# blyssprivacy/sdk

Measured on AMD Instinct MI355X. Metric: PIR queries/sec (full answer path) on 2^20 items x 256 B, higher is better.
Workload: dtype u64; 1 GPU; spiral-rs process_query, c2 = {"db_item_size": 256, "instances": 1, "n": 2, "nu_1": 9, "nu_2": 11, "p": 256, "q2_bits": 20, "t_conv": 4, "t_exp_left": 8, "t_exp_right": 56, "t_gsw": 8}, encoded DB 64.0 GiB (56.0 GiB resident per GPU), unsharded, one query per step

## Files before the change

### sdk_amd/csrc/capi.cpp

```cpp
#include <chrono>
#include <cstdlib>
#include <cstring>
#include <deque>
#include <new>

#include "../../include/spiral_hip.h"
#include "pipeline.hpp"

using namespace spiral;

static thread_local std::string g_last_error;
static thread_local int g_last_rc = SP_OK;

template <typename F>
static int guarded(F&& f) {
  tunables_new_call();
  auto fail = [](int rc, const char* what) {
    g_last_error = what;
    g_last_rc = rc;
    return rc;
  };
  try {
    f();
    g_last_rc = SP_OK;
// ... 226 lines not shown
  }
  auto idx = std::make_shared<SparseIndex>();
  idx->col_ptr.ensure(ptr.size());
  idx->col_rows.ensure(std::max<size_t>(rows.size(), 1));
  idx->col_slots.ensure(std::max<size_t>(slots.size(), 1));
  upload_words(idx->col_ptr.p, ptr.data(), ptr.size() * sizeof(int));
  if (!rows.empty()) {
    upload_words(idx->col_rows.p, rows.data(), rows.size() * sizeof(int));
    upload_words(idx->col_slots.p, slots.data(), slots.size() * sizeof(int));
  }
  if (slots_cap == 0) polys.ensure(1);
  if (rows_dirty || !sparse_index || !sparse_index->plan)
    idx->plan = build_pruned_plan_rows(p, row_set);
  else
    idx->plan = sparse_index->plan;
  sparse_index = idx;
  index_dirty = false;
  rows_dirty = false;
  return sparse_index;
}

extern "C" {

const char* sp_last_error(void) { return g_last_error.c_str(); }

uint64_t sp_paths_taken(int reset) { return paths_taken(reset != 0); }
int sp_debug_set(const char* name, long value) {
  if (!name) return SP_E_ARG;
  set_tunable(name, value);
  return SP_OK;
}
static thread_local int g_shard_split_hint = 1;
extern "C" void sp_shard_split_hint_(int on) { g_shard_split_hint = on; }
extern "C" int sp_scatter_group_choice_(const sp_db_t* db, int G) {
  if (!db || !db->packed || db->col_G != 1 || db->sparse || db->num_shards != G) return 1;
  SweepBatchDesc d{};
  d.batch = SWEEP_BATCH_MAX;
  d.num_per = db->np_local;
  d.nj = db->nj;
  tunables_new_call();
  return sweep_batch_scatter_ok(d, G) && G <= (int)tunable("batch_scatter_max_g", BATCH_SCATTER_MAX_G_DEFAULT) ? SWEEP_BATCH_MAX : 1;
}
void sp_set_last_error_(const char* msg) { g_last_error = msg ? msg : ""; }
void sp_note_path_(uint64_t bits) { note_path(bits); }

const char* sp_path_name(int bit) {
  static const char* names[] = {"sweep_packed_persist", "sweep_packed", "sweep_wide", "sweep_narrow", "sweep_batch",
                                "from_sweep4", "from_sweep1", "fold_fused", "fold_tail_delta", "fold_tail_literal",
                                "pipelined_fold_overlap", "expand_pruned", "pack_v1", "direct_upload", "scatter_out",
                                "from_sweep4_xcd_order", "fold_tail_persistent", "expand_round_one_launch", "sweep_sparse",
                                "rccl_in_library", "fold_wave", "cu_split_overlap", "expand_split", "pipe_class_split",
                                "sweep_batch_mfma", "custom_transport", "from_sweep_wave",
                                "fold_tail_batched", "sweep_ring", "sweep_batch_mfma_two_tiles", "fold_wave8", "sweep_batch_planar",
                                "expand_group", "expand_wave", "sweep_batch_scatter"};
  return bit >= 0 && bit < (int)(sizeof(names) / sizeof(names[0])) ? names[bit] : nullptr;
}

int sp_device_count(void) {
  int n = 0;
  if (hipGetDeviceCount(&n) != hipSuccess) {
    (void)hipGetLastError();
    return 0;
  }
  return n;
}
int sp_set_device(int device) {
  return guarded([&] { HIP_CHECK(hipSetDevice(device)); });
}

sp_params_t* sp_params_from_json(const char* json) {
  sp_params_t* out = nullptr;
  int rc = guarded([&] {
    need(json != nullptr, "json is null");
    auto h = std::make_unique<sp_params>();
    h->p = Params::from_json(json);
    out = h.release();
  });
  return rc == SP_OK ? out : nullptr;
}
void sp_params_free(sp_params_t* p) { delete p; }

uint64_t sp_params_get(const sp_params_t* h, const char* name) {
  if (!h || !name) return UINT64_MAX;
  const Params& p = h->p;
  std::string s(name);
  if (s == "poly_len") return p.poly_len;
  if (s == "poly_len_log2") return p.poly_len_log2;
  if (s == "crt_count") return p.crt_count;
  if (s == "modulus") return p.modulus;
  if (s == "modulus_log2") return p.modulus_log2;
  if (s == "moduli0") return p.moduli[0];
  if (s == "moduli1") return p.moduli[1];
  if (s == "n") return p.n;
  if (s == "pt_modulus") return p.pt_modulus;
  if (s == "q2_bits") return p.q2_bits;
  if (s == "t_conv") return p.t_conv;
  if (s == "t_exp_left") return p.t_exp_left;
  if (s == "t_exp_right") return p.t_exp_right;
  if (s == "t_gsw") return p.t_gsw;
  if (s == "expand_queries") return p.expand_queries;
  if (s == "db_dim_1") return p.db_dim_1;
  if (s == "db_dim_2") return p.db_dim_2;
  if (s == "instances") return p.instances;
  if (s == "db_item_size") return p.db_item_size;
  if (s == "version") return p.version;
  if (s == "g") return p.g();
  if (s == "stop_round") return p.stop_round();
// ... 1353 lines not shown
    join_right(*W);
    download_raw(*W, W->qv.p, POLY_LEN * p.dim0() * 2, v_reg_reoriented);
    const size_t nu2 = p.db_dim_2, two_t = 2 * p.t_gsw;
    if (nu2 > 0) {
      need(v_folding != nullptr, "v_folding is null");
      DevBuf<u32> dense(nu2 * 2 * two_t * 2 * POLY_LEN);
      for (size_t d = 0; d < nu2; d++)
        for (size_t r = 0; r < 2; r++)
          HIP_CHECK(hipMemcpyAsync(dense.p + ((d * 2 + r) * two_t) * 2 * POLY_LEN,
                                   W->fold_mats.p + ((d * 2 + r) * 2 * two_t + two_t) * 2 * POLY_LEN,
                                   two_t * 2 * POLY_LEN * sizeof(u32), hipMemcpyDeviceToDevice, W->stream));
      DevBuf<u64> tmp;
      download_ntt(*W, dense.p, nu2 * 2 * two_t * 2 * POLY_LEN, v_folding, tmp);
    }
  });
}

int sp_fold_ciphertexts(const sp_params_t* h, uint64_t* cts, size_t num_per, const uint64_t* v_folding,
                        const uint64_t* v_folding_neg) {
  return guarded([&] {
    need(h && cts && v_folding && v_folding_neg, "null argument");
    const Params& p = h->p;
    need(num_per >= 1 && (num_per & (num_per - 1)) == 0, "num_per must be a power of two");
    size_t further = 0;
    while (((size_t)1 << further) < num_per) further++;
    if (further == 0) return;
    const size_t two_t = 2 * p.t_gsw;
    Scoped W(h);
    ensure_stage_fold(*W, num_per, further);
    DevBuf<u64> tmp;
    DevBuf<u32> dF, dFn;
    upload_ntt(*W, v_folding, further * 2 * two_t * 2 * POLY_LEN, dF, tmp);
    DevBuf<u64> tmp2;
    upload_ntt(*W, v_folding_neg, further * 2 * two_t * 2 * POLY_LEN, dFn, tmp2);
    for (size_t d = 0; d < further; d++)
      for (size_t r = 0; r < 2; r++) {
        u32* row = W->fold_mats.p + ((d * 2 + r) * 2 * two_t) * 2 * POLY_LEN;
        HIP_CHECK(hipMemcpyAsync(row, dFn.p + ((d * 2 + r) * two_t) * 2 * POLY_LEN, two_t * 2 * POLY_LEN * sizeof(u32), hipMemcpyDeviceToDevice, W->stream));
        HIP_CHECK(hipMemcpyAsync(row + two_t * 2 * POLY_LEN, dF.p + ((d * 2 + r) * two_t) * 2 * POLY_LEN, two_t * 2 * POLY_LEN * sizeof(u32), hipMemcpyDeviceToDevice, W->stream));
      }
    HIP_CHECK(hipMemcpyAsync(W->foldX.p, cts, num_per * 2 * POLY_LEN * 8, hipMemcpyHostToDevice, W->stream));
    W->mats_w_ready = false;
    u64* res = run_fold(*W, FoldOpts{1L << 60, false, false}, W->foldX.p, W->foldY.p, 1, (int)num_per, -1);
    download_raw(*W, res, 2 * POLY_LEN, cts);
  });
}

int sp_fold_ciphertexts_fused(const sp_params_t* h, uint64_t* cts, size_t num_per, const uint64_t* v_folding,
                              long fused_min_pairs) {
  return guarded([&] {
    need(h && cts && v_folding, "null argument");
    const Params& p = h->p;
    need(num_per >= 1 && (num_per & (num_per - 1)) == 0, "num_per must be a power of two");
    size_t further = 0;
    while (((size_t)1 << further) < num_per) further++;
    if (further == 0) return;
    const size_t two_t = 2 * p.t_gsw;
    Scoped W(h);
    ensure_stage_fold(*W, num_per, further);
    DevBuf<u64> tmp;
    DevBuf<u32> dF;
    upload_ntt(*W, v_folding, further * 2 * two_t * 2 * POLY_LEN, dF, tmp);
    for (size_t d = 0; d < further; d++)
      for (size_t r = 0; r < 2; r++) {
        u32* row = W->fold_mats.p + ((d * 2 + r) * 2 * two_t) * 2 * POLY_LEN;
        HIP_CHECK(hipMemcpyAsync(row + two_t * 2 * POLY_LEN, dF.p + ((d * 2 + r) * two_t) * 2 * POLY_LEN, two_t * 2 * POLY_LEN * sizeof(u32), hipMemcpyDeviceToDevice, W->stream));
      }
    launch_folding_neg(W->D->T, W->fold_mats.p, W->D->gadget_gsw.p, (int)further, (int)two_t, W->stream);
    run_mats_to_wave(*W, further);
    HIP_CHECK(hipMemcpyAsync(W->foldX.p, cts, num_per * 2 * POLY_LEN * 8, hipMemcpyHostToDevice, W->stream));
    bool below_q = true;
    for (size_t i = 0; i < num_per * 2 * POLY_LEN && below_q; i++) below_q = cts[i] < p.modulus;
    const FoldOpts o{fused_min_pairs > 0 ? fused_min_pairs : W->fused_min_pairs, true, below_q};
    u64* res = run_fold(*W, o, W->foldX.p, W->foldY.p, 1, (int)num_per, -1);
    download_raw(*W, res, 2 * POLY_LEN, cts);
  });
}

int sp_pack(const sp_params_t* h, const sp_pp_t* pp, const uint64_t* v_ct, uint64_t* out) {
  return guarded([&] {
    need(h && pp && v_ct && out, "null argument");
    const Params& p = h->p;
    need(p.instances == 1, "sp_pack packs one instance (n*n cts); call per instance");
    check_device(pp->device);
    Scoped W(h);
    W->ensure_finish();
    HIP_CHECK(hipMemcpyAsync(W->final_cts.p, v_ct, p.n * p.n * 2 * POLY_LEN * 8, hipMemcpyHostToDevice, W->stream));
    run_pack(*W, *pp);
    DevBuf<u64> tmp;
    download_ntt(*W, W->pack_res.p, (p.n + 1) * p.n * 2 * POLY_LEN, out, tmp);
  });
}

int sp_encode(const sp_params_t* h, const uint64_t* v_packed, uint8_t* out, size_t out_cap, size_t* out_len) {
  return guarded([&] {
    need(h && v_packed && out && out_len, "null argument");
    need(out_cap >= h->p.response_bytes(), "output buffer smaller than response_bytes");
    *out_len = encode_response(h->p, v_packed, out);
  });
}

}
```

### sdk_amd/csrc/fold.hip

```cpp
#include <type_traits>

#include "device_common.hpp"
#include "wave_ntt.hpp"
#include "bodies.hpp"

namespace spiral {

__device__ __forceinline__ bool fold_zero_shortcut(const u64* ct0, const u64* ct1, u64* out, int tau) {
  int nz0 = 0, nz1 = 0;
#pragma unroll
  for (int k = 0; k < 16; k++) {
    nz0 |= ct0[tau + 256 * k] != 0;
    nz1 |= ct1[tau + 256 * k] != 0;
  }
  const int any0 = __syncthreads_or(nz0), any1 = __syncthreads_or(nz1);
  if (any0 && any1) return false;
  const u64* src = any0 ? ct0 : ct1;
#pragma unroll
  for (int k = 0; k < 16; k++) out[tau + 256 * k] = src[tau + 256 * k];
  return true;
}

__global__ __launch_bounds__(256, 2) void k_fold_fused(DevTables T, FoldDesc d) {
  __shared__ u32 lds0[LDS_WORDS];
  __shared__ u32 lds1[LDS_WORDS];
  const int tau = threadIdx.x;
  const int i = (int)blockIdx.x, plane = blockIdx.y;
  const int two_t = 2 * d.t, four_t = 4 * d.t;
  const int t_live = d.t_live > 0 && d.t_live < d.t ? d.t_live : d.t;
  const u64* ct0 = d.X + ((size_t)plane * d.cur + i) * 2 * N;
  const u64* ct1 = ct0 + (size_t)d.half * 2 * N;
  const u64 mask = (1ULL << d.bits) - 1ULL;
  u32* la = lds0;
  u32* lb = lds1;
  u64* out = d.Y + ((size_t)plane * d.half + i) * 2 * N;
  if (d.zero_shortcuts && fold_zero_shortcut(ct0, ct1, out, tau)) return;
#pragma unroll 1
  for (int c = 0; c < 2; c++) {
    const ModConst m = T.c.mod[c];
    const u32* fw = T.tw + (size_t)c * 4 * N;
    u64 acc0[8], acc1[8];
#pragma unroll
    for (int k = 0; k < 8; k++) acc0[k] = acc1[k] = 0;
#pragma unroll 1
    for (int j = 0; j < 2; j++) {
      u64 x0[8], x1[8];
#pragma unroll
      for (int k = 0; k < 8; k++) {
        x0[k] = ct0[(size_t)j * N + tau + 256 * k];
        x1[k] = ct1[(size_t)j * N + tau + 256 * k];
      }
#pragma unroll 1
// ... 371 lines not shown
#pragma unroll
        for (int k = 0; k < 32; k++) rr[k] = wv == 0 ? r0[k] : r1[k];
      } else {
#pragma unroll
        for (int g = 0; g < 8; g++) {
          const u32x4w_t t4 = *reinterpret_cast<const u32x4w_t*>(park + irow * N + g * 256 + 4 * lt);
          rr[4 * g] = t4.x; rr[4 * g + 1] = t4.y; rr[4 * g + 2] = t4.z; rr[4 * g + 3] = t4.w;
        }
      }
      const int khalf = wv >> 1;
      const u64* crow = ct0 + (size_t)irow * N + (size_t)khalf * 1024;
      u64 cpre[16];
#pragma unroll
      for (int kk = 0; kk < 16; kk++) cpre[kk] = crow[64 * kk + lt];
      wntt_inv(rr, lt, mybuf, inv_tables(T.tw, imod), mi.q, mi.two_q);
      u32* exch = smem_fw + 4 * WBUF_WORDS;
      u32* mine_out = exch + (irow * 2 + imod) * (N / 2);
      if (wv < 2) {
#pragma unroll
        for (int kk = 0; kk < 16; kk++) mine_out[64 * kk + lt] = rr[16 + kk];
      } else {
#pragma unroll
        for (int kk = 0; kk < 16; kk++) mine_out[64 * kk + lt] = rr[kk];
      }
      __syncthreads();
      {
        const u32* theirs = exch + (irow * 2 + (1 - imod)) * (N / 2);
        u64* orow = out + (size_t)irow * N + (size_t)khalf * 1024;
        const u32 q0 = T.c.mod[0].q, q1 = T.c.mod[1].q;
        auto compose = [&](auto mod1_wave) {
          constexpr bool M1 = decltype(mod1_wave)::value;
#pragma unroll
          for (int kk = 0; kk < 16; kk++) {
            const u32 other = theirs[64 * kk + lt];
            const u32 own = rr[M1 ? kk : 16 + kk];
            const u32 x = M1 ? other : own, y = M1 ? own : other;
            const u32 xm = x >= q1 ? x - q1 : x;
            const u32 dd = y >= xm ? y - xm : y + q1 - xm;
            const u32 qt = __umulhi(dd, T.c.q0_inv_q1_sh);
            u32 e = dd * T.c.q0_inv_q1 - qt * q1;
            e = e >= q1 ? e - q1 : e;
            const u64 val = (u64)x + (u64)q0 * (u64)e + cpre[kk];
            const u64 res = val >= T.c.Q ? val - T.c.Q : val;
            orow[64 * kk + lt] = res;
          }
        };
        if (wv < 2) compose(std::true_type{});
        else compose(std::false_type{});
      }
    }
  }
}

__global__ __launch_bounds__(256, 2) void k_expand_wave(DevTables T, ExpandWaveDesc d, GroupOff g) {
  extern __shared__ __attribute__((aligned(16))) u32 smem_fw[];
  u32* wbuf = smem_fw;
  u32* ltw = smem_fw + 4 * WBUF_WORDS;
  u64* raw0 = reinterpret_cast<u64*>(ltw + 2 * N);
  const int tau = threadIdx.x, lane = tau & 63;
  const int wv = __builtin_amdgcn_readfirstlane(tau >> 6);
  const int b = (int)blockIdx.x, c = (int)blockIdx.y, qi = (int)blockIdx.z;
  const ModConst m = T.c.mod[c];
  const u32* fw = T.tw + (size_t)c * 4 * N;
  const u64* src = group_rebase(d.raw, g.raw[qi]) + (size_t)d.pos[b] * 2 * N;
  const u32* A_w = group_rebase(d.A_w, g.pp[qi]);
  u32* vout = group_rebase(d.v, g.v[qi]);
  u32* mybuf = wbuf + wv * WBUF_WORDS;
  wtw_stage(ltw, wave_fwd_image(T.tw, c), tau);
#pragma unroll
  for (int k = 0; k < 8; k++) raw0[tau + 256 * k] = src[tau + 256 * k];
  __syncthreads();
  const u64 mask = (1ULL << d.bits) - 1ULL;
  u64 acc0[32], acc1[32];
#pragma unroll
  for (int k = 0; k < 32; k++) acc0[k] = acc1[k] = 0;
#pragma unroll 1
  for (int dg = wv; dg <= d.t; dg += 4) {
    int ln = lane;
    const u32* fwi = fw;
    asm volatile("" : "+v"(ln));
    asm volatile("" : "+s"(fwi));
    WaveScalarTw stw;
    wntt_scalar_tw(stw, fwi);
    u32 v[32];
    if (dg < d.t) {
      const int sh = dg * d.bits;
#pragma unroll
      for (int k = 0; k < 32; k++) v[k] = sh < 64 ? (u32)((raw0[64 * k + ln] >> (sh & 63)) & mask) : 0u;
    } else {
#pragma unroll
      for (int k = 0; k < 32; k++) v[k] = reduce64(src[(size_t)N + 64 * k + ln], m);
    }
    SP_SB();
    const u32* a0 = dg < d.t ? A_w + ((size_t)dg * 2 + c) * N : d.const_w;
    const u32* a1 = dg < d.t ? A_w + ((size_t)(d.t + dg) * 2 + c) * N : d.const_w + N;
    FoldMac hk{acc0, acc1, reinterpret_cast<const u32x4w_t*>(a0) + ln, reinterpret_cast<const u32x4w_t*>(a1) + ln};
    wntt_fwd<false>(v, ln, mybuf, fwi, stw, ltw, m.q, m.two_q, hk);
  }
  int lt = lane;
  asm volatile("" : "+v"(lt));
  u32 r0[32], r1[32];
#pragma unroll
  for (int k = 0; k < 32; k++) {
    r0[k] = reduce64(acc0[k], m);
    r1[k] = reduce64(acc1[k], m);
  }
// ... 97 lines not shown
```

### sdk_amd/csrc/kernels.hpp

```cpp
#pragma once
#include <hip/hip_runtime.h>

#include <vector>

#include "params.hpp"

namespace spiral {

constexpr int N = (int)POLY_LEN;

struct DevTables {
  const u32* tw;
  DevConsts c;
};
__host__ __device__ inline const u32* inv_tables(const u32* tw, int c) { return tw + (size_t)8 * N + (size_t)c * 2 * N; }
__host__ __device__ inline const u32* wave_fwd_image(const u32* tw, int c) { return tw + (size_t)12 * N + (size_t)c * 2 * N; }
__host__ __device__ inline int wtw_phys(int idx) {
  if (idx >= 1024) {
    const int L = (idx - 1024) >> 4, r = (idx - 1024) & 15;
    return 1024 + 16 * L + 4 * (((r >> 2) + (L >> 2)) & 3) + (r & 3);
  }
  if (idx >= 512) {
    const int L = (idx - 512) >> 3, r = (idx - 512) & 7;
    return 512 + 8 * L + 4 * (((r >> 2) + (L >> 3)) & 1) + (r & 3);
  }
  return idx;
}

enum PathBit : u64 {
  PATH_SWEEP_PERSIST = 1ull << 0,
  PATH_SWEEP_PACKED = 1ull << 1,
  PATH_SWEEP_WIDE = 1ull << 2,
  PATH_SWEEP_NARROW = 1ull << 3,
  PATH_SWEEP_BATCH = 1ull << 4,
  PATH_FROM_SWEEP4 = 1ull << 5,
  PATH_FROM_SWEEP1 = 1ull << 6,
  PATH_FOLD_FUSED = 1ull << 7,
  PATH_FOLD_TAIL = 1ull << 8,
  PATH_FOLD_TAIL_LITERAL = 1ull << 9,
  PATH_PIPELINED = 1ull << 10,
  PATH_EXPAND_PRUNED = 1ull << 11,
  PATH_PACK_V1 = 1ull << 12,
  PATH_DIRECT_UPLOAD = 1ull << 13,
  PATH_SCATTER_OUT = 1ull << 14,
  PATH_SWEEP_XCD_FROM = 1ull << 15,
  PATH_FOLD_TAIL_PERSIST = 1ull << 16,
  PATH_EXPAND_FUSED = 1ull << 17,
  PATH_SWEEP_SPARSE = 1ull << 18,
  PATH_RCCL = 1ull << 19,
  PATH_FOLD_WAVE = 1ull << 20,
  PATH_CU_SPLIT = 1ull << 21,
  PATH_EXPAND_SPLIT = 1ull << 22,
  PATH_PIPE_CLASS_SPLIT = 1ull << 23,
  PATH_SWEEP_MFMA = 1ull << 24,
  PATH_CUSTOM_TRANSPORT = 1ull << 25,
  PATH_FROM_SWEEP_WAVE = 1ull << 26,
  PATH_FOLD_TAIL_BATCHED = 1ull << 27,
  PATH_SWEEP_RING = 1ull << 28,
  PATH_SWEEP_MFMA2 = 1ull << 29,
  PATH_FOLD_WAVE8 = 1ull << 30,
  PATH_SWEEP_PLANAR = 1ull << 31,
  PATH_EXPAND_GROUP = 1ull << 32,
  PATH_EXPAND_WAVE = 1ull << 33,
  PATH_SWEEP_BATCH_SCATTER = 1ull << 34
};
long tunable(const char* name, long dflt);
void launched(u64 path_bits, const char* kernel);
void note_path(u64 path_bits);
void launch_checksum(const u32* p, size_t n_words, unsigned long long* out, hipStream_t s);
void launch_cache_sync(u32* sink, hipStream_t s);
void launch_copy_words(u32* dst, const u32* src, size_t n_words, hipStream_t s);
void debug_stage(int stage);

struct FwdDesc {
  const u64* src;
  const int* src_idx;
  u32* dst;
  int n_out;
  int rdim, cols, t, bits;
  int src_batch_stride;
  int src_row0, src_cols;
  long delta_off;
  int delta_inner, delta_outer_stride;
};
void launch_ntt_fwd(const DevTables& T, const FwdDesc& d, hipStream_t s);
void launch_ntt_fwd3(const DevTables& T, const FwdDesc& d0, const FwdDesc& d1, const FwdDesc& d2, hipStream_t s);

float bench_ntt_core(const DevTables& T, int M, int blocks, int reps, u32* scratch, hipStream_t s);

struct InvDesc {
  const u32* src;
  const int* idx;
  int polys_per_idx;
  long idx_stride, poly_stride, crt_stride, z_stride;
  u64* dst;
  int n_polys;
  int premod;
  int sweep_np;
  int automorph_t;
  const u32* scal;
  u32* scal_dst;
  int scal_thresh;
  const int* scal_only_idx;
  int n_scalar_only;
  const u64* addend;
  int add_inner2, add_outer_stride;
};
void launch_ntt_inv(const DevTables& T, const InvDesc& d, hipStream_t s);
void launch_from_sweep4(const DevTables& T, const u32* src, int np, int n_planes, int premod, u64* dst, hipStream_t s);

struct MacDesc {
  const u32* A;
  const u32* B;
  u32* out;
  const u32* addend;
  const int* out_idx;
  int R, K;
// ... 13 lines not shown
struct ExpandSideDesc {
  const u64* raw;
  const int* pos;
  const int* out_idx;
  const u32* A;
  u32* v;
  int cnt, t, bits;
};
void launch_expand_round(const DevTables& T, const ExpandSideDesc& left, const ExpandSideDesc& right, hipStream_t s);
constexpr long EXPAND_ROUND_MIN_DEFAULT = 2048;

constexpr int GROUP_MAX = 16;
struct GroupOff {
  long long v[GROUP_MAX], raw[GROUP_MAX], dig[GROUP_MAX], ct1[GROUP_MAX], pp[GROUP_MAX];
};
void launch_ntt_inv_group(const DevTables& T, const InvDesc& d, const GroupOff& g, int B, hipStream_t s);
void launch_ntt_fwd3_group(const DevTables& T, const FwdDesc& d0, const FwdDesc& d1, const FwdDesc& d2, const GroupOff& g, int B,
                           hipStream_t s);
void launch_mac2_group(const DevTables& T, const MacDesc& d0, const MacDesc& d1, const GroupOff& g, int B, hipStream_t s);
void launch_expand_round_group(const DevTables& T, const ExpandSideDesc& left, const ExpandSideDesc& right, const GroupOff& g, int B,
                               hipStream_t s);
void launch_reorient_group(u64* out, const u32* v, int first, int step, int dim0, const GroupOff& g, int B, hipStream_t s);
void launch_copy_polys_group(u32* dst, const int* dst_idx, int dst_row_stride, const u32* src, const int* src_idx, int src_row_stride,
                             int R, int batch, const GroupOff& g, int B, hipStream_t s);
void launch_folding_neg_group(const DevTables& T, u32* mats, const u32* gadget_ntt, int nu2, int two_t, const GroupOff& g, int B,
                              hipStream_t s);
void launch_mats_to_wave_group(u32* dst, const u32* src, size_t n_words, int half_polys, const GroupOff& g, int B, hipStream_t s);
struct ExpandWaveDesc {
  const u64* raw;
  const int* pos;
  const int* out_idx;
  const u32* A_w;
  const u32* const_w;
  u32* v;
  int cnt, t, bits;
};
void launch_expand_wave(const DevTables& T, const ExpandWaveDesc& d, const GroupOff& g, int B, hipStream_t s);
constexpr long EXPAND_WAVE_MIN_DIGITS_DEFAULT = 16;
constexpr long EXPAND_GROUP_ROUND_MIN_DEFAULT = 4096;

struct FoldDesc {
  const u64* X;
  u64* Y;
  const u32* mats;
  int cur, half, planes;
  int t, bits;
  int t_live;
  int zero_shortcuts;
  const u32* mats_w;
};
void launch_mats_to_wave(u32* dst, const u32* src, size_t n_words, hipStream_t s, int half_polys = 0);
constexpr long FOLD_VARIANT_DEFAULT = 5;
void launch_fold_fused(const DevTables& T, const FoldDesc& d, hipStream_t s);

void launch_add_poly_into(const DevTables& T, u32* dst, const int* idx, const u32* src, int batch, hipStream_t s);
void launch_scalar_mul(const DevTables& T, u32* base, long dst_off, long src_off, const u32* scalar, int n_polys,
                       hipStream_t s);
void launch_add_polys_idx(const DevTables& T, u32* dst, const int* di, const u32* a, const int* ai, const u32* b,
                          const int* bi, int count, hipStream_t s);
void launch_interleave_query(u64* qv, const u32* row0_ntt, const u64* wire, int dim0, hipStream_t s);
void launch_copy_polys(u32* dst, const int* dst_idx, int dst_row_stride, const u32* src, const int* src_idx,
                       int src_row_stride, int R, int batch, hipStream_t s);
void launch_folding_neg(const DevTables& T, u32* mats, const u32* gadget_ntt, int nu2, int two_t, hipStream_t s);
void launch_add(const DevTables& T, u32* out, const u32* a, const u32* b, int n_polys, hipStream_t s);
void launch_invert_raw(const DevTables& T, u64* out, const u64* a, long n_words, hipStream_t s);
void launch_automorph(const DevTables& T, u64* out, const u64* a, int n_polys, int t, hipStream_t s);
void launch_gadget_raw(u64* out, const u64* inp, int rows_in, int cols, int rows_out, int rdim, int bits,
                       hipStream_t s);
void launch_u64_to_u32(u32* out, const u64* in, long n, hipStream_t s);
void launch_u32_to_u64(u64* out, const u32* in, long n, hipStream_t s);

void launch_cu_probe(u32* out, int blocks, hipStream_t s);

struct EncodeDesc {
  const u64* packed;
  unsigned long long* out;
  int instances, n;
  u64 Q, q1, q2;
  int q1_bits, q2_bits;
};
void launch_encode(const EncodeDesc& d, hipStream_t s);

void launch_reorient(u64* out, const u32* v, int first, int step, int dim0, hipStream_t s);

struct CopyPolysDesc {
  u32* dst;
  const int* dst_idx;
  int dst_row_stride;
  const u32* src;
  const int* src_idx;
  int src_row_stride, R, batch;
};
struct FoldingNegDesc {
  u32* mats;
  const u32* gadget_ntt;
  int two_t, nu2;
};
struct ReorientDesc {
  u64* out;
  const u32* v;
  int first, step, dim0;
};
struct MatsToWaveDesc {
  u32* dst;
  const u32* src;
  size_t n_words;
// ... 103 lines not shown
```

### sdk_amd/csrc/pipeline.hpp

```cpp
#pragma once
#include <vector>

#include "server.hpp"

namespace spiral {

struct Workspace {
  const Params* P;
  DeviceState* D;
  int device = -1;
  hipStream_t stream = nullptr;
  hipStream_t stream2 = nullptr;
  std::vector<hipEvent_t> ev_plane;
  hipEvent_t ev_fold = nullptr;
  hipEvent_t ev_round0 = nullptr, ev_right = nullptr;
  bool right_pending = false;
  bool long_sweep_follows = false;
  hipEvent_t ev_sw[2] = {nullptr, nullptr};
  bool have_sweep_span = false;
  bool pipelined = false;
  hipEvent_t ev[5] = {nullptr, nullptr, nullptr, nullptr, nullptr};
  DevBuf<u64> q_raw;
  DevBuf<u32> v;
  DevBuf<u64> exp_raw;
// ... 9 lines not shown
  DevBuf<u32> gsw_dig;
  DevBuf<u32> sweep_out;
  DevBuf<u64> fold_tail;
  DevBuf<u32> batch_rq;
  DevBuf<u64> foldX, foldY, final_cts, pack_raw;
  DevBuf<u32> fold_dig, fold_ntt, pack_dig, pack_ct2, pack_res, pack_v1_P, pack_v1_P2;
  DevBuf<u64> pack_v1_raw, du_raw, du_wire;
  DevBuf<u32> du_ntt;
  u64* h_query = nullptr;
  u64* h_group_query = nullptr;
  DevBuf<u64> group_q_raw;
  u64* h_packed = nullptr;
  size_t h_packed_words = 0;
  DevBuf<u64> enc_out;
  uint8_t* h_response = nullptr;
  bool host_pinned = true;
  int out_G = 1;
  bool zero_shortcuts = false;
  long fused_min_pairs = 256;

  Workspace(const Params& P, DeviceState& D);
  ~Workspace();
  Workspace(const Workspace&) = delete;
  Workspace& operator=(const Workspace&) = delete;
  void ensure_expand();
  void ensure_sweep();
  void ensure_finish();
  size_t plane_group() const;
};

void run_coefficient_expansion(Workspace& W, const sp_pp& pp, size_t g_rounds, const DeviceState::PrunedPlan* plan = nullptr,
                               int tree = 0, size_t r_begin = 0);
void join_right(Workspace& W);
void run_regev_to_gsw(Workspace& W, const sp_pp& pp, const u32* v_src, const int* src_ct, const int* src_poly);
void run_folding_neg(Workspace& W);
void run_mats_to_wave(Workspace& W, size_t levels, bool c_only = false);
void run_fold_operands(Workspace& W);
void run_begin_direct(Workspace& W, const uint8_t* query);
void run_begin_group(Workspace* const* Ws, const sp_pp* const* pps, const uint8_t* const* queries, const size_t* query_lens, int B);
void run_begin(Workspace& W, const sp_pp& pp, const uint8_t* query, size_t query_len, int j0 = 0, int nj = 0,
               const DeviceState::PrunedPlan* plan = nullptr);
void run_sweep_sparse(Workspace& W, const sp_db& db, const int* col_ptr, const int* col_rows, const int* col_slots);
std::unique_ptr<DeviceState::PrunedPlan> build_pruned_plan_rows(const Params& P, const std::vector<char>& rows);
void run_sweep(Workspace& W, const sp_db& db);
void run_sweep_pipelined(Workspace& W, const sp_db& db);
bool sweep_is_pipelined(const Params& p, const sp_db& db);
void launch_plane_sweep(Workspace& W, const sp_db& db, size_t plane);
bool fused_fold_supported(const Params& p);
struct FoldOpts {
  long fused_min_pairs;
  bool delta_tail;
  bool inputs_below_q;
};
u64* run_fold(Workspace& W, const FoldOpts& o, u64* X, u64* Y, int np, int num_cts, int top, int d_begin = 0, int d_end = -1);
void run_fold_local(Workspace& W, const u32* reduced_chunk, int G);
void run_fold_local_plane(Workspace& W, const u32* reduced_plane_chunk, int G, int plane);
void run_fold_local_join(Workspace& W);
void run_finish_gathered(Workspace& W, const sp_pp& pp, const u64* gathered, int G);
void run_fold_all(Workspace& W, bool premod);
void run_pack(Workspace& W, const sp_pp& pp);
void run_finish(Workspace& W, const sp_pp& pp, bool premod);
size_t encode_response(const Params& p, const u64* packed, uint8_t* out);
void run_encode_device(Workspace& W);

}
```

### sdk_amd/csrc/server.cpp

```cpp
#include "server.hpp"

#include <algorithm>
#include <atomic>
#include <cstdlib>
#include <cstring>
#include <functional>

#include "pipeline.hpp"

namespace spiral {

void hip_check(hipError_t e, const char* what, const char* file, int line) {
  if (e != hipSuccess) {
    (void)hipGetLastError();
    throw HipError(std::string(what) + " failed at " + file + ":" + std::to_string(line) + ": " + hipGetErrorString(e));
  }
}

static std::mutex g_tun_mu;
static std::vector<std::pair<std::string, long>> g_tun;
static std::atomic<unsigned> g_tun_epoch{1};
static std::atomic<long> g_fresh_allocs{0};
void tunables_new_call() { g_tun_epoch.fetch_add(1, std::memory_order_relaxed); }
void set_tunable(const char* name, long v) {
// ... 1098 lines not shown
      run_coefficient_expansion(W, pp, g, pl, 2, 1);
      run_regev_to_gsw(W, pp, W.v.p, L + D.gsw_src_ct, L + D.gsw_src_poly);
      run_fold_operands(W);
    });
    HIP_CHECK(hipEventRecord(W.ev_right, W.stream2));
    W.right_pending = true;
    run_coefficient_expansion(W, pp, g, pl, 1, 1);
    launch_reorient(W.qv.p, W.v.p, 0, 2, (int)p.dim0(), s);
    return;
  }
  run_coefficient_expansion(W, pp, g, pl);
  run_begin_after_rounds(W, pp);
}

void join_right(Workspace& W) {
  if (W.right_pending) HIP_CHECK(hipStreamWaitEvent(W.stream, W.ev_right, 0));
}

void run_sweep(Workspace& W, const sp_db& db) {
  const Params& p = *W.P;
  W.ensure_sweep();
  SweepDesc d{db.words.p, W.qv.p, W.sweep_out.p, (int)p.planes(), db.np_local, (int)p.dim0(), db.j0, db.nj, db.packed, W.out_G};
  d.nt_store = (int)tunable("sweep_nt_store", 1);
  launch_sweep(W.D->T, d, W.stream);
}

void run_sweep_sparse(Workspace& W, const sp_db& db, const int* col_ptr, const int* col_rows, const int* col_slots) {
  const Params& p = *W.P;
  W.ensure_sweep();
  launch_sweep_sparse(W.D->T, col_ptr, col_rows, col_slots, db.polys.p, (int)p.planes(), W.v.p, 0,
                      p.db_dim_2 > 0 ? 2 : 1, W.sweep_out.p, (int)p.num_per(), W.stream);
}

static FoldOpts query_fold_opts(const Workspace& W, bool below_q) {
  return FoldOpts{std::min(W.fused_min_pairs, tunable("fused_min_pairs_cap", 1L << 62)), true, below_q};
}

static void fold_planes(Workspace& W, size_t pg0, int np, bool premod) {
  const Params& p = *W.P;
  DeviceState& D = *W.D;
  hipStream_t s = W.stream;
  if (p.num_per() % 4 == 0 && !tunable("from_sweep1", 0)) {
    launch_from_sweep4(D.T, W.sweep_out.p + pg0 * 4 * POLY_LEN * p.num_per(), (int)p.num_per(), np, premod ? 1 : 0,
                       W.foldX.p, s);
  } else {
    InvDesc inv{};
    inv.src = W.sweep_out.p + pg0 * 4 * POLY_LEN * p.num_per();
    inv.sweep_np = (int)p.num_per();
    inv.dst = W.foldX.p;
    inv.n_polys = np * (int)p.num_per() * 2;
    inv.premod = premod ? 1 : 0;
    launch_ntt_inv(D.T, inv, s);
  }
  u64* res = run_fold(W, query_fold_opts(W, true), W.foldX.p, W.foldY.p, np, (int)p.num_per(), -1);
  HIP_CHECK(hipMemcpyAsync(W.final_cts.p + pg0 * 2 * POLY_LEN, res, (size_t)np * 2 * POLY_LEN * sizeof(u64), hipMemcpyDeviceToDevice, s));
}

static int tail_defer_levels(const Params& p, long stop) {
  if (stop <= 0 || !fused_fold_supported(p) || p.planes() < 2) return 0;
  int lv = 0;
  size_t cur = p.num_per();
  while (cur > (size_t)stop && cur / 2 >= 1 && (cur & 1) == 0) { cur >>= 1; lv++; }
  return cur == (size_t)stop && lv > 0 && stop >= 2 ? lv : 0;
}
static void fold_plane_head(Workspace& W, size_t pl, int levels) {
  const Params& p = *W.P;
  launch_from_sweep4(W.D->T, W.sweep_out.p + pl * 4 * POLY_LEN * p.num_per(), (int)p.num_per(), 1, 0, W.foldX.p, W.stream);
  u64* res = run_fold(W, query_fold_opts(W, true), W.foldX.p, W.foldY.p, 1, (int)p.num_per(), -1, 0, levels);
  const size_t cts = p.num_per() >> levels;
  HIP_CHECK(hipMemcpyAsync(W.fold_tail.p + pl * cts * 2 * POLY_LEN, res, cts * 2 * POLY_LEN * sizeof(u64), hipMemcpyDeviceToDevice, W.stream));
}
static void fold_tails(Workspace& W, int levels) {
  const Params& p = *W.P;
  const size_t cts = p.num_per() >> levels;
  u64* other = W.fold_tail.p + p.planes() * cts * 2 * POLY_LEN;
  u64* res = run_fold(W, query_fold_opts(W, true), W.fold_tail.p, other, (int)p.planes(), (int)p.num_per(), -1, levels, -1);
  HIP_CHECK(hipMemcpyAsync(W.final_cts.p, res, p.planes() * 2 * POLY_LEN * sizeof(u64), hipMemcpyDeviceToDevice, W.stream));
}

bool sweep_is_pipelined(const Params& p, const sp_db& db) {
  const bool enabled = tunable("pipeline", 1) != 0;
  return enabled && db.packed && db.num_shards == 1 && db.col_G == 1 && p.planes() > 1 && p.num_per() >= 1024;
}

void launch_plane_sweep(Workspace& W, const sp_db& db, size_t pl) {
  const Params& p = *W.P;
  const size_t np_ = (size_t)db.np_local;
  const size_t plane_db_words = db_bytes(1, db.np_local, db.nj, db.packed) / 8;
  SweepDesc d{db.words.p + pl * plane_db_words, W.qv.p, W.sweep_out.p + pl * 4 * POLY_LEN * np_, 1, db.np_local,
              (int)p.dim0(), db.j0, db.nj, db.packed, W.out_G};
  d.nt_store = (int)tunable("sweep_nt_store", 1);
  const int wgs = (int)tunable("pipe_wgs", 4);
  if (db.packed && wgs > 0)
    launch_sweep_persist(W.D->T, d, wgs, W.stream);
  else
    launch_sweep(W.D->T, d, W.stream);
}

void run_sweep_pipelined(Workspace& W, const sp_db& db) {
  const Params& p = *W.P;
  W.ensure_sweep();
  W.ensure_finish();
  const size_t planes = p.planes();
  HIP_CHECK(hipEventRecord(W.ev_sw[0], W.stream));
  const int defer_levels = tail_defer_levels(p, tunable("pipe_tail_defer", 256));
  if (defer_levels > 0) {
    W.fold_tail.ensure(2 * planes * (p.num_per() >> defer_levels) * 2 * POLY_LEN);
    note_path(PATH_FOLD_TAIL_BATCHED);
  }
  for (size_t pl = 0; pl < planes; pl++) {
    launch_plane_sweep(W, db, pl);
    HIP_CHECK(hipEventRecord(W.ev_plane[pl], W.stream));
    HIP_CHECK(hipStreamWaitEvent(W.stream2, W.ev_plane[pl], 0));
    if (defer_levels > 0) {
      on_stream(W, W.stream2, [&] {
        fold_plane_head(W, pl, defer_levels);
        if (pl + 1 == planes) fold_tails(W, defer_levels);
      });
      continue;
    }
    on_stream(W, W.stream2, [&] { fold_planes(W, pl, 1, false); });
  }
  HIP_CHECK(hipEventRecord(W.ev_sw[1], W.stream));
  HIP_CHECK(hipEventRecord(W.ev_fold, W.stream2));
  W.have_sweep_span = true;
  W.pipelined = true;
  note_path(PATH_PIPELINED);
}

bool fused_fold_supported(const Params& p) { return 4 * p.t_gsw <= 128 && p.bits_per(p.t_gsw) <= 28; }

u64* run_fold(Workspace& W, const FoldOpts& o, u64* X, u64* Y, int np, int num_cts, int top, int d_begin, int d_end) {
  const Params& p = *W.P;
  DeviceState& D = *W.D;
  hipStream_t s = W.stream;
  const int two_t = (int)(2 * p.t_gsw);
  join_right(W);
  int further = 0;
  while (((int)1 << further) < num_cts) further++;
  const int top_idx = top < 0 ? further - 1 : top;
  if (d_end < 0) d_end = further;
  int cur = num_cts >> d_begin;
  for (int d = d_begin; d < d_end; d++) {
    const int half = cur / 2;
    if (W.zero_shortcuts && !fused_fold_supported(p))
      throw ArgError("sparse buckets need gadget parameters the fused fold supports (3 <= t_gsw <= 32)");
    if (W.zero_shortcuts || ((long)np * half >= o.fused_min_pairs && fused_fold_supported(p))) {
      FoldDesc fd{};
      fd.zero_shortcuts = W.zero_shortcuts ? 1 : 0;
      fd.mats_w = W.mats_w_ready ? W.fold_mats_w.p + (size_t)(top_idx - d) * 2 * 2 * two_t * 2 * POLY_LEN : nullptr;
      fd.X = X;
      fd.Y = Y;
      fd.mats = W.fold_mats.p + (size_t)(top_idx - d) * 2 * 2 * two_t * 2 * POLY_LEN;
      fd.cur = cur;
      fd.half = half;
      fd.planes = np;
      fd.t = (int)p.t_gsw;
      fd.bits = (int)p.bits_per(p.t_gsw);
      fd.t_live = o.inputs_below_q && tunable("fold_skip_dead_digits", 1)
                      ? (int)std::min<size_t>(p.t_gsw, (p.modulus_log2 + fd.bits - 1) / fd.bits) : fd.t;
      launch_fold_fused(D.T, fd, s);
      std::swap(X, Y);
      cur = half;
      continue;
    }
    if (o.delta_tail) {
      FwdDesc f{};
      f.src = X;
      f.dst = W.fold_dig.p;
      f.n_out = np * half * two_t;
      f.rdim = 2;
      f.cols = 1;
      f.t = (int)p.t_gsw;
      f.bits = (int)p.bits_per(p.t_gsw);
      f.src_batch_stride = 2;
      f.src_row0 = 0;
      f.src_cols = 1;
      f.delta_off = (long)half * 2;
      f.delta_inner = half;
      f.delta_outer_stride = cur;
      launch_ntt_fwd(D.T, f, s);
      MacDesc m{};
      m.A = W.fold_mats.p + ((size_t)(top_idx - d) * 2 * 2 * two_t + two_t) * 2 * POLY_LEN;
      m.A_row_stride = 2 * two_t;
      m.B = W.fold_dig.p;
      m.out = W.fold_ntt.p;
      m.R = 2;
      m.K = two_t;
      m.batch_inner = np * half;
      m.batch_outer = 1;
      m.B_inner_stride = two_t;
      m.split_k = two_t;
      m.out_batch_stride = 2;
      m.out_row_stride = 1;
      launch_mac(D.T, m, s);
      InvDesc inv{};
      inv.src = W.fold_ntt.p;
      inv.poly_stride = 2 * POLY_LEN;
      inv.crt_stride = POLY_LEN;
      inv.z_stride = 1;
      inv.dst = Y;
      inv.n_polys = np * half * 2;
      inv.addend = X;
      inv.add_inner2 = half * 2;
      inv.add_outer_stride = cur * 2;
      launch_ntt_inv(D.T, inv, s);
      note_path(PATH_FOLD_TAIL);
      std::swap(X, Y);
      cur = half;
      continue;
    }
    FwdDesc f{};
    f.src = X;
    f.dst = W.fold_dig.p;
// ... 302 lines not shown
```

Before: 92.75 queries/s.

## Add single-launch fold tail kernel and write final fold level into destination

```diff
diff --git a/sdk_amd/csrc/capi.cpp b/sdk_amd/csrc/capi.cpp
--- a/sdk_amd/csrc/capi.cpp
+++ b/sdk_amd/csrc/capi.cpp
@@ -302,7 +302,7 @@
                                 "rccl_in_library", "fold_wave", "cu_split_overlap", "expand_split", "pipe_class_split",
                                 "sweep_batch_mfma", "custom_transport", "from_sweep_wave",
                                 "fold_tail_batched", "sweep_ring", "sweep_batch_mfma_two_tiles", "fold_wave8", "sweep_batch_planar",
-                                "expand_group", "expand_wave", "sweep_batch_scatter"};
+                                "expand_group", "expand_wave", "sweep_batch_scatter", "fold_tail_one_launch"};
   return bit >= 0 && bit < (int)(sizeof(names) / sizeof(names[0])) ? names[bit] : nullptr;
 }
 
@@ -1762,8 +1762,11 @@
     need(h && cts && v_folding, "null argument");
     const Params& p = h->p;
     need(num_per >= 1 && (num_per & (num_per - 1)) == 0, "num_per must be a power of two");
+    const size_t planes = (size_t)std::max(1L, tunable("stage_fold_planes", 1));
+    need((planes & (planes - 1)) == 0 && planes <= num_per, "stage_fold_planes must be a power of two <= num_per");
+    const size_t per = num_per / planes;
     size_t further = 0;
-    while (((size_t)1 << further) < num_per) further++;
+    while (((size_t)1 << further) < per) further++;
     if (further == 0) return;
     const size_t two_t = 2 * p.t_gsw;
     Scoped W(h);
@@ -1782,8 +1785,8 @@
     bool below_q = true;
     for (size_t i = 0; i < num_per * 2 * POLY_LEN && below_q; i++) below_q = cts[i] < p.modulus;
     const FoldOpts o{fused_min_pairs > 0 ? fused_min_pairs : W->fused_min_pairs, true, below_q};
-    u64* res = run_fold(*W, o, W->foldX.p, W->foldY.p, 1, (int)num_per, -1);
-    download_raw(*W, res, 2 * POLY_LEN, cts);
+    u64* res = run_fold(*W, o, W->foldX.p, W->foldY.p, (int)planes, (int)per, -1);
+    download_raw(*W, res, planes * 2 * POLY_LEN, cts);
   });
 }
 
diff --git a/sdk_amd/csrc/fold.hip b/sdk_amd/csrc/fold.hip
--- a/sdk_amd/csrc/fold.hip
+++ b/sdk_amd/csrc/fold.hip
@@ -1,3 +1,4 @@
+#include <stdexcept>
 #include <type_traits>
 
 #include "device_common.hpp"
@@ -475,6 +476,222 @@
   }
 }
 
+constexpr int FOLD_TAIL_FIXED_LDS = (8 * WBUF_WORDS + 4 * N) * 4;
+constexpr size_t FOLD_TAIL_MAX_LDS = 160 * 1024;
+
+template <int ES>
+__global__ __launch_bounds__(512) void k_fold_tail(DevTables T, FoldDesc d, const u32* __restrict__ mats_w) {
+  extern __shared__ __attribute__((aligned(16))) u32 smem_fw[];
+  u32* wbuf = smem_fw;
+  u32* ltw2 = smem_fw + 8 * WBUF_WORDS;
+  const int t_live = d.t_live > 0 && d.t_live < d.t ? d.t_live : d.t;
+  unsigned char* dig = reinterpret_cast<unsigned char*>(ltw2 + 4 * N);
+  unsigned char* sgn = dig + (size_t)2 * t_live * (N * ES);
+  constexpr int E = 16 / ES;
+  const int tau = threadIdx.x, lane = tau & 63;
+  const int wv = __builtin_amdgcn_readfirstlane(tau >> 6);
+  const int c = wv >> 2, w4 = wv & 3;
+  const int i = (int)blockIdx.x, plane = blockIdx.y;
+  const int two_t = 2 * d.t, four_t = 4 * d.t;
+  const u64* ct0 = d.X + ((size_t)plane * d.cur + i) * 2 * N;
+  const u64* ct1 = ct0 + (size_t)d.half * 2 * N;
+  u64* out = d.Y + ((size_t)plane * d.half + i) * 2 * N;
+  u32* mybuf = wbuf + wv * WBUF_WORDS;
+  {
+    const int j = c, kq = w4;
+    const u64 mask = (1ULL << d.bits) - 1ULL;
+    u64 x0[8], x1[8];
+#pragma unroll
+    for (int e = 0; e < 8; e++) {
+      const size_t n = (size_t)j * N + 64 * (8 * kq + e) + lane;
+      x0[e] = ct0[n];
+      x1[e] = ct1[n];
+    }
+#pragma unroll
+    for (int k = 0; k < 4; k++)
+      reinterpret_cast<u32x4w_t*>(ltw2)[tau + 512 * k] = reinterpret_cast<const u32x4w_t*>(wave_fwd_image(T.tw, 0))[tau + 512 * k];
+#pragma unroll 1
+    for (int kd = 0; kd < t_live; kd++) {
+      const int sh = (kd * d.bits) & 63;
+      const u64 dmask = kd * d.bits >= 64 ? 0ULL : mask;
+      u32 df[8];
+#pragma unroll
+      for (int e = 0; e < 8; e++) df[e] = (u32)((x1[e] >> sh) & dmask) - (u32)((x0[e] >> sh) & dmask);
+      unsigned char* base = dig + (size_t)(j * t_live + kd) * (N * ES);
+      u32 sb = 0;
+#pragma unroll
+      for (int e = 0; e < 8; e++) sb |= (df[e] >> 31) << e;
+      sgn[(j * t_live + kd) * 256 + lane * 4 + kq] = (unsigned char)sb;
+      if (ES == 1) {
+        u32x2w_t o;
+        o.x = (df[0] & 0xff) | ((df[1] & 0xff) << 8) | ((df[2] & 0xff) << 16) | (df[3] << 24);
+        o.y = (df[4] & 0xff) | ((df[5] & 0xff) << 8) | ((df[6] & 0xff) << 16) | (df[7] << 24);
+        *reinterpret_cast<u32x2w_t*>(base + (kq >> 1) * 1024 + lane * 16 + 8 * (kq & 1)) = o;
+      } else if (ES == 2) {
+        u32x4w_t o;
+        o.x = (df[0] & 0xffff) | (df[1] << 16); o.y = (df[2] & 0xffff) | (df[3] << 16);
+        o.z = (df[4] & 0xffff) | (df[5] << 16); o.w = (df[6] & 0xffff) | (df[7] << 16);
+        *reinterpret_cast<u32x4w_t*>(base + kq * 1024 + lane * 16) = o;
+      } else {
+        u32x4w_t o;
+        o.x = df[0]; o.y = df[1]; o.z = df[2]; o.w = df[3];
+        *reinterpret_cast<u32x4w_t*>(base + (2 * kq) * 1024 + lane * 16) = o;
+        o.x = df[4]; o.y = df[5]; o.z = df[6]; o.w = df[7];
+        *reinterpret_cast<u32x4w_t*>(base + (2 * kq + 1) * 1024 + lane * 16) = o;
+      }
+    }
+  }
+  const ModConst m = T.c.mod[c];
+  const u32* fw = T.tw + (size_t)c * 4 * N;
+  const u32* ltw = ltw2 + c * 2 * N;
+  __syncthreads();
+  u64 acc0[32], acc1[32];
+#pragma unroll
+  for (int k = 0; k < 32; k++) acc0[k] = acc1[k] = 0;
+  const int wv0 = (w4 + 2 * c) & 3;
+#pragma unroll 1
+  for (int dg = wv0; dg < 2 * t_live; dg += 4) {
+    const int j = dg / t_live, kd = dg - j * t_live;
+    int ln = lane;
+    const u32* fwi = fw;
+    asm volatile("" : "+v"(ln));
+    asm volatile("" : "+s"(fwi));
+    const unsigned char* src = dig + (size_t)dg * (N * ES) + ln * 16;
+    u32x4w_t dv[2 * ES];
+#pragma unroll
+    for (int h = 0; h < 2 * ES; h++) dv[h] = *reinterpret_cast<const u32x4w_t*>(src + h * 1024);
+    const int sg = *reinterpret_cast<const int*>(sgn + dg * 256 + ln * 4);
+    WaveScalarTw stw;
+    wntt_scalar_tw(stw, fwi);
+    SP_SB();
+    u32 v[32];
+#pragma unroll
+    for (int h = 0; h < 2 * ES; h++) {
+      const u32 wd[4] = {dv[h].x, dv[h].y, dv[h].z, dv[h].w};
+#pragma unroll
+      for (int e = 0; e < E; e++) {
+        const int sm = __builtin_amdgcn_sbfe(sg, h * E + e, 1);
+        const int sd = ES == 4 ? (int)wd[e] : (int)(__builtin_amdgcn_ubfe(wd[(e * ES) >> 2], ((e * ES) & 3) * 8, 8 * ES) | ((u32)sm << (8 * ES)));
+        u32 x = (u32)(sd + (sm & (int)m.q));
+        if (ES == 4) {
+          x += (u32)(((int)x >> 31) & (int)m.q);
+          x -= (x >= m.q ? m.q : 0u);
+        }
+        v[h * E + e] = x;
+      }
+    }
+    const int kk = two_t + j + 2 * kd;
+    FoldMac hk{acc0, acc1, reinterpret_cast<const u32x4w_t*>(mats_w + ((size_t)kk * 2 + c) * N) + ln,
+               reinterpret_cast<const u32x4w_t*>(mats_w + ((size_t)(four_t + kk) * 2 + c) * N) + ln};
+    wntt_fwd<false>(v, ln, mybuf, fwi, stw, ltw, m.q, m.two_q, hk);
+  }
+  int lt = lane;
+  asm volatile("" : "+v"(lt));
+  u32 r0[32], r1[32];
+#pragma unroll
+  for (int k = 0; k < 32; k++) {
+    r0[k] = reduce64(acc0[k], m);
+    r1[k] = reduce64(acc1[k], m);
+  }
+  u32x4w_t* sc = reinterpret_cast<u32x4w_t*>(smem_fw) + c * 2048;
+#define SP_PUT(R, REGION)                                                                              \
+_Pragma("unroll") for (int g = 0; g < 8; g++) {                                                      \
+  u32x4w_t t4;                                                                                       \
+  t4.x = R[4 * g]; t4.y = R[4 * g + 1]; t4.z = R[4 * g + 2]; t4.w = R[4 * g + 3];                    \
+  sc[(REGION) * 512 + g * 64 + lt] = t4;                                                             \
+}
+#define SP_ADD(R, REGION)                                                                              \
+_Pragma("unroll") for (int g = 0; g < 8; g++) {                                                      \
+  const u32x4w_t t4 = sc[(REGION) * 512 + g * 64 + lt];                                              \
+  R[4 * g] = add_mod(R[4 * g], t4.x, m.q); R[4 * g + 1] = add_mod(R[4 * g + 1], t4.y, m.q);          \
+  R[4 * g + 2] = add_mod(R[4 * g + 2], t4.z, m.q); R[4 * g + 3] = add_mod(R[4 * g + 3], t4.w, m.q);  \
+}
+  __syncthreads();
+  if (w4 == 2) { SP_PUT(r0, 0) SP_PUT(r1, 1) }
+  if (w4 == 3) { SP_PUT(r0, 2) SP_PUT(r1, 3) }
+  __syncthreads();
+  if (w4 == 0) { SP_ADD(r0, 0) SP_ADD(r0, 2) }
+  if (w4 == 1) { SP_ADD(r1, 1) SP_ADD(r1, 3) }
+  __syncthreads();
+  if (w4 == 0) { SP_PUT(r1, 0) }
+  if (w4 == 1) { SP_PUT(r0, 1) }
+  __syncthreads();
+  if (w4 == 0) { SP_ADD(r0, 1) }
+  if (w4 == 1) { SP_ADD(r1, 0) }
+  __syncthreads();
+#undef SP_PUT
+#undef SP_ADD
+  const bool act = w4 < 2;
+  const int irow = w4 & 1, khalf = 1 - c;
+  u32 rr[32];
+#pragma unroll
+  for (int k = 0; k < 32; k++) rr[k] = w4 == 0 ? r0[k] : r1[k];
+  const u64* crow = ct0 + (size_t)irow * N + (size_t)khalf * 1024;
+  u64 cpre[16];
+#pragma unroll
+  for (int kk = 0; kk < 16; kk++) cpre[kk] = act ? crow[64 * kk + lt] : 0ULL;
+  u32* exch = ltw2;
+  if (act) {
+    wntt_inv(rr, lt, mybuf, inv_tables(T.tw, c), m.q, m.two_q);
+    u32* mine_out = exch + (irow * 2 + c) * (N / 2);
+    if (c == 1) {
+#pragma unroll
+      for (int kk = 0; kk < 16; kk++) mine_out[64 * kk + lt] = rr[16 + kk];
+    } else {
+#pragma unroll
+      for (int kk = 0; kk < 16; kk++) mine_out[64 * kk + lt] = rr[kk];
+    }
+  }
+  __syncthreads();
+  if (act) {
+    const u32* theirs = exch + (irow * 2 + (1 - c)) * (N / 2);
+    u64* orow = out + (size_t)irow * N + (size_t)khalf * 1024;
+    const u32 q0 = T.c.mod[0].q, q1 = T.c.mod[1].q;
+    auto compose = [&](auto mod1_wave) {
+      constexpr bool M1 = decltype(mod1_wave)::value;
+#pragma unroll
+      for (int kk = 0; kk < 16; kk++) {
+        const u32 other = theirs[64 * kk + lt];
+        const u32 own = rr[M1 ? kk : 16 + kk];
+        const u32 x = M1 ? other : own, y = M1 ? own : other;
+        const u32 xm = x >= q1 ? x - q1 : x;
+        const u32 dd = y >= xm ? y - xm : y + q1 - xm;
+        const u32 qt = __umulhi(dd, T.c.q0_inv_q1_sh);
+        u32 e = dd * T.c.q0_inv_q1 - qt * q1;
+        e = e >= q1 ? e - q1 : e;
+        const u64 val = (u64)x + (u64)q0 * (u64)e + cpre[kk];
+        const u64 res = val >= T.c.Q ? val - T.c.Q : val;
+        orow[64 * kk + lt] = res;
+      }
+    };
+    if (c == 1) compose(std::true_type{});
+    else compose(std::false_type{});
+  }
+}
+
+static int fold_digit_es(const FoldDesc& d) { return d.bits <= 8 ? 1 : d.bits <= 16 ? 2 : 4; }
+static size_t fold_tail_lds(const FoldDesc& d) {
+  const int t_live = d.t_live > 0 && d.t_live < d.t ? d.t_live : d.t;
+  return FOLD_TAIL_FIXED_LDS + (size_t)2 * t_live * (N * fold_digit_es(d) + 256);
+}
+bool fold_tail_takes(const FoldDesc& d) {
+  return d.mats_w && !d.zero_shortcuts && d.bits <= 28 && fold_tail_lds(d) <= FOLD_TAIL_MAX_LDS;
+}
+void launch_fold_tail(const DevTables& T, const FoldDesc& d, hipStream_t s) {
+  if (d.half <= 0 || d.planes <= 0) return;
+  if (!fold_tail_takes(d)) throw std::runtime_error("launch_fold_tail: shape not taken by k_fold_tail");
+  const dim3 grid(d.half, d.planes), block(512);
+  const size_t lds = fold_tail_lds(d);
+  const int es = fold_digit_es(d);
+  if (es == 1)
+    hipLaunchKernelGGL(k_fold_tail<1>, grid, block, lds, s, T, d, d.mats_w);
+  else if (es == 2)
+    hipLaunchKernelGGL(k_fold_tail<2>, grid, block, lds, s, T, d, d.mats_w);
+  else
+    hipLaunchKernelGGL(k_fold_tail<4>, grid, block, lds, s, T, d, d.mats_w);
+  launched(PATH_FOLD_TAIL_ONE_LAUNCH, "k_fold_tail");
+}
+
 __global__ __launch_bounds__(256, 2) void k_expand_wave(DevTables T, ExpandWaveDesc d, GroupOff g) {
   extern __shared__ __attribute__((aligned(16))) u32 smem_fw[];
   u32* wbuf = smem_fw;
diff --git a/sdk_amd/csrc/kernels.hpp b/sdk_amd/csrc/kernels.hpp
--- a/sdk_amd/csrc/kernels.hpp
+++ b/sdk_amd/csrc/kernels.hpp
@@ -62,7 +62,8 @@
   PATH_SWEEP_PLANAR = 1ull << 31,
   PATH_EXPAND_GROUP = 1ull << 32,
   PATH_EXPAND_WAVE = 1ull << 33,
-  PATH_SWEEP_BATCH_SCATTER = 1ull << 34
+  PATH_SWEEP_BATCH_SCATTER = 1ull << 34,
+  PATH_FOLD_TAIL_ONE_LAUNCH = 1ull << 35
 };
 long tunable(const char* name, long dflt);
 void launched(u64 path_bits, const char* kernel);
@@ -182,6 +183,9 @@
 void launch_mats_to_wave(u32* dst, const u32* src, size_t n_words, hipStream_t s, int half_polys = 0);
 constexpr long FOLD_VARIANT_DEFAULT = 5;
 void launch_fold_fused(const DevTables& T, const FoldDesc& d, hipStream_t s);
+constexpr long FOLD_TAIL_ONE_LAUNCH_DEFAULT = 0;
+bool fold_tail_takes(const FoldDesc& d);
+void launch_fold_tail(const DevTables& T, const FoldDesc& d, hipStream_t s);
 
 void launch_add_poly_into(const DevTables& T, u32* dst, const int* idx, const u32* src, int batch, hipStream_t s);
 void launch_scalar_mul(const DevTables& T, u32* base, long dst_off, long src_off, const u32* scalar, int n_polys,
diff --git a/sdk_amd/csrc/pipeline.hpp b/sdk_amd/csrc/pipeline.hpp
--- a/sdk_amd/csrc/pipeline.hpp
+++ b/sdk_amd/csrc/pipeline.hpp
@@ -85,7 +85,8 @@
   bool delta_tail;
   bool inputs_below_q;
 };
-u64* run_fold(Workspace& W, const FoldOpts& o, u64* X, u64* Y, int np, int num_cts, int top, int d_begin = 0, int d_end = -1);
+u64* run_fold(Workspace& W, const FoldOpts& o, u64* X, u64* Y, int np, int num_cts, int top, int d_begin = 0, int d_end = -1,
+              u64* last_dst = nullptr);
 void run_fold_local(Workspace& W, const u32* reduced_chunk, int G);
 void run_fold_local_plane(Workspace& W, const u32* reduced_plane_chunk, int G, int plane);
 void run_fold_local_join(Workspace& W);
diff --git a/sdk_amd/csrc/server.cpp b/sdk_amd/csrc/server.cpp
--- a/sdk_amd/csrc/server.cpp
+++ b/sdk_amd/csrc/server.cpp
@@ -1174,8 +1174,10 @@
     inv.premod = premod ? 1 : 0;
     launch_ntt_inv(D.T, inv, s);
   }
-  u64* res = run_fold(W, query_fold_opts(W, true), W.foldX.p, W.foldY.p, np, (int)p.num_per(), -1);
-  HIP_CHECK(hipMemcpyAsync(W.final_cts.p + pg0 * 2 * POLY_LEN, res, (size_t)np * 2 * POLY_LEN * sizeof(u64), hipMemcpyDeviceToDevice, s));
+  u64* dst = W.final_cts.p + pg0 * 2 * POLY_LEN;
+  u64* res = run_fold(W, query_fold_opts(W, true), W.foldX.p, W.foldY.p, np, (int)p.num_per(), -1, 0, -1, dst);
+  if (res != dst)
+    HIP_CHECK(hipMemcpyAsync(dst, res, (size_t)np * 2 * POLY_LEN * sizeof(u64), hipMemcpyDeviceToDevice, s));
 }
 
 static int tail_defer_levels(const Params& p, long stop) {
@@ -1188,16 +1190,14 @@
 static void fold_plane_head(Workspace& W, size_t pl, int levels) {
   const Params& p = *W.P;
   launch_from_sweep4(W.D->T, W.sweep_out.p + pl * 4 * POLY_LEN * p.num_per(), (int)p.num_per(), 1, 0, W.foldX.p, W.stream);
-  u64* res = run_fold(W, query_fold_opts(W, true), W.foldX.p, W.foldY.p, 1, (int)p.num_per(), -1, 0, levels);
   const size_t cts = p.num_per() >> levels;
-  HIP_CHECK(hipMemcpyAsync(W.fold_tail.p + pl * cts * 2 * POLY_LEN, res, cts * 2 * POLY_LEN * sizeof(u64), hipMemcpyDeviceToDevice, W.stream));
+  run_fold(W, query_fold_opts(W, true), W.foldX.p, W.foldY.p, 1, (int)p.num_per(), -1, 0, levels, W.fold_tail.p + pl * cts * 2 * POLY_LEN);
 }
 static void fold_tails(Workspace& W, int levels) {
   const Params& p = *W.P;
   const size_t cts = p.num_per() >> levels;
   u64* other = W.fold_tail.p + p.planes() * cts * 2 * POLY_LEN;
-  u64* res = run_fold(W, query_fold_opts(W, true), W.fold_tail.p, other, (int)p.planes(), (int)p.num_per(), -1, levels, -1);
-  HIP_CHECK(hipMemcpyAsync(W.final_cts.p, res, p.planes() * 2 * POLY_LEN * sizeof(u64), hipMemcpyDeviceToDevice, W.stream));
+  run_fold(W, query_fold_opts(W, true), W.fold_tail.p, other, (int)p.planes(), (int)p.num_per(), -1, levels, -1, W.final_cts.p);
 }
 
 bool sweep_is_pipelined(const Params& p, const sp_db& db) {
@@ -1252,7 +1252,7 @@
 
 bool fused_fold_supported(const Params& p) { return 4 * p.t_gsw <= 128 && p.bits_per(p.t_gsw) <= 28; }
 
-u64* run_fold(Workspace& W, const FoldOpts& o, u64* X, u64* Y, int np, int num_cts, int top, int d_begin, int d_end) {
+u64* run_fold(Workspace& W, const FoldOpts& o, u64* X, u64* Y, int np, int num_cts, int top, int d_begin, int d_end, u64* last_dst) {
   const Params& p = *W.P;
   DeviceState& D = *W.D;
   hipStream_t s = W.stream;
@@ -1263,12 +1263,14 @@
   const int top_idx = top < 0 ? further - 1 : top;
   if (d_end < 0) d_end = further;
   int cur = num_cts >> d_begin;
+  const bool fused_ok = fused_fold_supported(p);
   for (int d = d_begin; d < d_end; d++) {
     const int half = cur / 2;
-    if (W.zero_shortcuts && !fused_fold_supported(p))
+    if (d + 1 == d_end && last_dst) Y = last_dst;
+    if (W.zero_shortcuts && !fused_ok)
       throw ArgError("sparse buckets need gadget parameters the fused fold supports (3 <= t_gsw <= 32)");
-    if (W.zero_shortcuts || ((long)np * half >= o.fused_min_pairs && fused_fold_supported(p))) {
-      FoldDesc fd{};
+    FoldDesc fd{};
+    if (fused_ok) {
       fd.zero_shortcuts = W.zero_shortcuts ? 1 : 0;
       fd.mats_w = W.mats_w_ready ? W.fold_mats_w.p + (size_t)(top_idx - d) * 2 * 2 * two_t * 2 * POLY_LEN : nullptr;
       fd.X = X;
@@ -1281,7 +1283,16 @@
       fd.bits = (int)p.bits_per(p.t_gsw);
       fd.t_live = o.inputs_below_q && tunable("fold_skip_dead_digits", 1)
                       ? (int)std::min<size_t>(p.t_gsw, (p.modulus_log2 + fd.bits - 1) / fd.bits) : fd.t;
+    }
+    if (W.zero_shortcuts || ((long)np * half >= o.fused_min_pairs && fused_ok)) {
       launch_fold_fused(D.T, fd, s);
+      std::swap(X, Y);
+      cur = half;
+      continue;
+    }
+    if (o.delta_tail && fused_ok && W.mats_w_ready && tunable("fold_tail_one_launch", FOLD_TAIL_ONE_LAUNCH_DEFAULT) != 0 &&
+        fold_tail_takes(fd)) {
+      launch_fold_tail(D.T, fd, s);
       std::swap(X, Y);
       cur = half;
       continue;
```

New measurement: 91.67 queries/s, median of 2. No clear change (-1.2%).
